# JakubValtar/basisu_rs

Measured on AMD Instinct MI355X. Metric: M 4x4 blocks/s UASTC->BC7 4096x4096, higher is better.
Workload: dtype u8

## Files before the change

basisu_rs_amd/csrc/bu_kernels.hpp:

```cpp
#pragma once
namespace {

constexpr unsigned bu_lds_front(int target) { return target == 1 ? (unsigned)sizeof(BuBc7Tables) : 0u; }
constexpr unsigned bu_lds_table_bytes(int target) { return bu_lds_front(target) + bu_table_bytes(target); }
template <int WGS, int TARGET>
__device__ __forceinline__ void bu_stage_tables_n(uint4* dst, const BuTablesAll* __restrict__ src)
{
    constexpr BuTableRange R = bu_table_range(TARGET);
    constexpr int F = (int)bu_lds_front(TARGET) / 16;
    const uint4* s = reinterpret_cast<const uint4*>(TARGET == 1 ? reinterpret_cast<const void*>(src) : reinterpret_cast<const void*>(&src->t));
    uint4* d = dst;
    for (int i = threadIdx.x; i < F + (int)(R.hi / 16); i += WGS)
        if (i < F || i >= F + (int)(R.lo / 16)) d[i] = s[i];
    if constexpr (R.lo2 < R.hi2) {
        for (int i = F + R.lo2 / 16 + threadIdx.x; i < F + (int)(R.hi2 / 16); i += WGS) d[i] = s[i];
    }
}

__device__ __forceinline__ void bu_report(unsigned long long* status, unsigned long long block, int st)
{
    if (status) (void)__hip_atomic_fetch_min(status, (block << 8) | (unsigned long long)st, __ATOMIC_RELAXED, __HIP_MEMORY_SCOPE_SYSTEM);
}

typedef unsigned int bu_v4u __attribute__((ext_vector_type(4)));
typedef unsigned int bu_v2u __attribute__((ext_vector_type(2)));
__device__ __forceinline__ uint4 bu_ld_stream(const uint4* p)
{
    const bu_v4u r = __builtin_nontemporal_load(reinterpret_cast<const bu_v4u*>(p));
    return make_uint4(r.x, r.y, r.z, r.w);
}
#ifndef BU_ST_MODE
#define BU_ST_MODE 4
#endif
#if BU_ST_MODE == 2
#define BU_ST_BITS " sc1"
#elif BU_ST_MODE == 3
#define BU_ST_BITS " sc0 sc1"
#elif BU_ST_MODE == 4
#define BU_ST_BITS " sc1 nt"
#endif
__device__ __forceinline__ void bu_st_stream(uint4* p, const uint4 v)
{
    bu_v4u r;
    r.x = v.x; r.y = v.y; r.z = v.z; r.w = v.w;
#if BU_ST_MODE == 0
    __builtin_nontemporal_store(r, reinterpret_cast<bu_v4u*>(p));
#elif BU_ST_MODE == 1
    *reinterpret_cast<bu_v4u*>(p) = r;
#else
    asm volatile("global_store_dwordx4 %0, %1, off" BU_ST_BITS "\n\ts_nop 1" ::"v"(p), "v"(r) : "memory");
#endif
}
__device__ __forceinline__ void bu_st_stream(uint2* p, const uint2 v)
{
    bu_v2u r;
    r.x = v.x; r.y = v.y;
#if BU_ST_MODE == 1
    *reinterpret_cast<bu_v2u*>(p) = r;
#else
    __builtin_nontemporal_store(r, reinterpret_cast<bu_v2u*>(p));
#endif
}

template <int TARGET>
__global__ __launch_bounds__(BU_WG) void bu_uastc_kernel(const uint4* __restrict__ in, void* __restrict__ out, size_t n_blocks,
                                                         unsigned bpr, unsigned long long base, unsigned long long* status,
                                                         const BuTablesAll* __restrict__ tables)
{
    __shared__ uint4 t_store[bu_lds_table_bytes(TARGET) / 16];
    BuTables& T = *reinterpret_cast<BuTables*>(t_store + bu_lds_front(TARGET) / 16);
    const size_t stride = (size_t)gridDim.x * BU_WG;
    size_t idx = (size_t)blockIdx.x * BU_WG + threadIdx.x;
    uint4 v = idx < n_blocks ? bu_ld_stream(in + idx) : make_uint4(0, 0, 0, 0);
    bu_stage_tables_n<BU_WG, TARGET>(t_store, tables);
    __syncthreads();
    while (idx < n_blocks) {
        const size_t next = idx + stride;
        const uint4 vn = next < n_blocks ? in[next] : make_uint4(0, 0, 0, 0);
        BuBlk b;
        b.w[0] = v.x;
        b.w[1] = v.y;
        b.w[2] = v.z;
        b.w[3] = v.w;
        const uint32_t mode = T.mode_lut[v.x & 127u];
        uint32_t o[TARGET == BU_TGT_RGBA ? 16 : 4];
#pragma unroll
        for (int i = 0; i < (TARGET == BU_TGT_RGBA ? 16 : 4); i++) o[i] = 0;
        const int st = bu_block_any<TARGET>(T, mode, b, o);
        if (st) {
            bu_report(status, base + idx, st);
#pragma unroll
            for (int i = 0; i < (TARGET == BU_TGT_RGBA ? 16 : 4); i++) o[i] = 0;
        }
        if constexpr (bu_out_words(TARGET) == 2) {
            reinterpret_cast<uint2*>(out)[idx] = make_uint2(o[0], o[1]);
        } else if constexpr (TARGET == BU_TGT_RGBA) {
            const size_t by = idx / bpr, bx = idx - by * bpr;
            uint4* img = reinterpret_cast<uint4*>(out);
#pragma unroll
            for (int r = 0; r < 4; r++) img[(4 * by + r) * (size_t)bpr + bx] = make_uint4(o[4 * r], o[4 * r + 1], o[4 * r + 2], o[4 * r + 3]);
        } else {
            reinterpret_cast<uint4*>(out)[idx] = make_uint4(o[0], o[1], o[2], o[3]);
        }
        v = vn;
        idx = next;
    }
}

__device__ __forceinline__ uint32_t bu_scan32(uint32_t v)
{
    v += (uint32_t)__builtin_amdgcn_update_dpp(0, (int)v, 0x111, 0xf, 0xf, false);
    v += (uint32_t)__builtin_amdgcn_update_dpp(0, (int)v, 0x112, 0xf, 0xf, false);
    v += (uint32_t)__builtin_amdgcn_update_dpp(0, (int)v, 0x114, 0xf, 0xf, false);
    v += (uint32_t)__builtin_amdgcn_update_dpp(0, (int)v, 0x118, 0xf, 0xf, false);
    v += (uint32_t)__builtin_amdgcn_update_dpp(0, (int)v, 0x142, 0xa, 0xf, false);
    return v;
}

struct BuRunDesc {
    const uint4* in;
    void* out;
    uint64_t base;
    uint32_t n;
    uint32_t vshift;
};
struct BuRunTable {
    BuRunDesc run[BU_MULTI_RUNS];
    uint32_t first_tile[BU_MULTI_RUNS + 32];
};
static_assert(sizeof(BuRunDesc) == 32 && sizeof(BuRunTable) <= 3968, "the run table must fit the 4 KiB of kernel arguments beside the other parameters");
struct BuTileDesc {
    const uint4* in;
    void* out;
    uint32_t first;
    uint32_t n;
    uint64_t base;
    uint32_t width;
};
enum { BU_LAYOUT_STRIP = 0, BU_LAYOUT_RECT = 1, BU_LAYOUT_MULTI = 2,
       BU_LAYOUT_MULTI_WHOLE = 3 };
constexpr unsigned BU_TICKET_STRIDE = 32, BU_TICKET_DONE = 8 * BU_TICKET_STRIDE, BU_TICKET_WORDS = 9 * BU_TICKET_STRIDE;
template <int TARGET, int WGS, int BPT, bool PREFETCH, int LAYOUT>
__device__ __forceinline__ void bu_uastc_sorted_body(const uint4* __restrict__ in, void* __restrict__ out, unsigned n_blocks,
                                                     unsigned bpr, unsigned long long base, unsigned long long* status,
                                                     const BuTablesAll* __restrict__ tables, unsigned cus, unsigned tile_rt,
                                                     const BuRunTable* __restrict__ runs, unsigned* __restrict__ ticket = nullptr)
{
    if (cus != 0) {
        constexpr bool ROT = TARGET == BU_TGT_BC7 || TARGET == BU_TGT_ASTC;
        if (blockIdx.x >= 3 * cus) __builtin_amdgcn_s_setprio(ROT ? 1 : 3);
        else if (blockIdx.x >= 2 * cus) __builtin_amdgcn_s_setprio(2);
        else if (blockIdx.x >= cus) __builtin_amdgcn_s_setprio(ROT ? 3 : 1);
    }
    constexpr int BU_WG = WGS, BU_BPT = BPT, BU_TILE = WGS * BPT;
    __shared__ uint4 t_store[bu_lds_table_bytes(TARGET) / 16];
    BuTables& T = *reinterpret_cast<BuTables*>(t_store + bu_lds_front(TARGET) / 16);
    constexpr bool RECT = LAYOUT == BU_LAYOUT_RECT, MULTI = LAYOUT == BU_LAYOUT_MULTI || LAYOUT == BU_LAYOUT_MULTI_WHOLE;
    constexpr bool WHOLE = RECT || LAYOUT == BU_LAYOUT_MULTI_WHOLE;
    constexpr bool BU_ALIAS = TARGET == BU_TGT_RGBA;
    static_assert(!BU_ALIAS || bu_lds_table_bytes(TARGET) + 4 * BU_TILE * 16 + BU_TILE + 1536 <= 80 * 1024,
                  "the RGBA32 workgroup no longer fits twice per CU: shrink BuTables or stage it per target in LDS too");
    __shared__ uint4 sblk_store[BU_ALIAS ? 1 : BU_TILE];
    __shared__ uint4 sout[BU_ALIAS ? 4 * BU_TILE : 1];
    uint4* const sblk = BU_ALIAS ? sout : sblk_store;
    constexpr bool INBLOCK = TARGET == BU_TGT_BC7 || TARGET == BU_TGT_ASTC;
    __shared__ uint8_t sst[INBLOCK ? 16 : BU_TILE];
    __shared__ uint32_t cnt[2][32], next_chunk[2];
    const unsigned tid = threadIdx.x, lane = tid & 63u;
    constexpr bool DYN_TILE = bu_dyn_tile(TARGET, BU_TILE) && LAYOUT != BU_LAYOUT_RECT;
    const unsigned tile_blocks = DYN_TILE ? tile_rt : (unsigned)BU_TILE;
    const unsigned n_tiles = (n_blocks + tile_blocks - 1) / tile_blocks;
    auto in_tile = [&](unsigned l) { return !DYN_TILE || l < tile_blocks; };
    static_assert(!RECT || BU_TILE % BU_RECT_W == 0, "rectangular tiles are BU_RECT_W blocks wide and of fixed size");
    const unsigned tpr = RECT ? bpr / BU_RECT_W : 1u;
    auto tile_xy = [&](unsigned t, unsigned& ty, unsigned& tx) {
        ty = (unsigned)(((unsigned long long)t * tile_rt) >> 32);
        tx = t - ty * tpr;
    };
    auto gidx = [&](unsigned t, unsigned l) {
        if constexpr (RECT) {
            unsigned ty, tx;
            tile_xy(t, ty, tx);
            return ((unsigned)(BU_TILE / BU_RECT_W) * ty + l / BU_RECT_W) * bpr + BU_RECT_W * tx + (l % BU_RECT_W);
        } else {
            return t * tile_blocks + l;
        }
    };
    auto has_block = [&](uint32_t k) { return WHOLE || k < 20u; };
    unsigned tile = blockIdx.x;
    __shared__ uint32_t s_next_tile[2];
    uint32_t my_draw = 0;
    unsigned* const my_counter = ticket ? ticket + (blockIdx.x & 7u) * BU_TICKET_STRIDE : nullptr;
    auto tile_of_draw = [&](uint32_t d) { return gridDim.x + 8u * d + (blockIdx.x & 7u); };
    if (ticket && tid == 0) my_draw = atomicAdd(my_counter, 1u);
    BuTileDesc td = {in, out, 0u, 0u, base, 0u}, tl = td;
    constexpr bool RUNS_IN_LDS = MULTI && PREFETCH;
    __shared__ uint4 s_runs[RUNS_IN_LDS ? sizeof(BuRunTable) / 16 : 1];
    const BuRunTable* R = runs;
    if constexpr (RUNS_IN_LDS) {
        static_assert(sizeof(BuRunTable) % 16 == 0, "copied in 16-byte pieces");
        for (unsigned i = tid; i < sizeof(BuRunTable) / 16; i += WGS) s_runs[i] = reinterpret_cast<const uint4*>(runs)[i];
    }
    auto uni32 = [](uint32_t x) { return (uint32_t)__builtin_amdgcn_readfirstlane((int)x); };
    auto uni64 = [&](uint64_t x) { return (uint64_t)uni32((uint32_t)x) | ((uint64_t)uni32((uint32_t)(x >> 32)) << 32); };
    auto desc_of = [&](unsigned t, BuTileDesc& d) {
        if constexpr (MULTI) {
            if (t < n_tiles) {
                uint32_t r = 0;
#pragma unroll
                for (unsigned c = 0; c < BU_MULTI_RUNS + 32; c += 64) {
                    const uint32_t cnt = (uint32_t)__popcll(__ballot(R->first_tile[c + lane] <= t));
                    if (cnt) r = c + cnt - 1u;
                }
                r = (uint32_t)__builtin_amdgcn_readfirstlane((int)r);
                const BuRunDesc rv = R->run[r];
                const BuRunDesc rd = {reinterpret_cast<const uint4*>(uni64(reinterpret_cast<uint64_t>(rv.in))), reinterpret_cast<void*>(uni64(reinterpret_cast<uint64_t>(rv.out))),
                                      uni64(rv.base), uni32(rv.n), uni32(rv.vshift)};
                const uint32_t lt = t - uni32(R->first_tile[r]);
                if (rd.vshift != BU_RUN_STRIPS) {
                    const uint32_t ty = lt >> rd.vshift, tx = lt & ((1u << rd.vshift) - 1u), width = (uint32_t)BU_RECT_W << rd.vshift;
                    d = BuTileDesc{rd.in, rd.out, (uint32_t)(BU_TILE / BU_RECT_W) * ty * width + (uint32_t)BU_RECT_W * tx, (uint32_t)BU_TILE, rd.base, width};
                } else {
                    const uint32_t first = lt * (uint32_t)BU_TILE, left = rd.n - first;
                    d = BuTileDesc{rd.in, rd.out, first, left < (uint32_t)BU_TILE ? left : (uint32_t)BU_TILE, rd.base, 0u};
                }
            }
        }
    };
    desc_of(tile, td);
    tl = td;
    auto run_idx = [&](const BuTileDesc& d, unsigned l) { return d.first + ((WHOLE || d.width) ? (l / BU_RECT_W) * d.width + (l % BU_RECT_W) : l); };
    auto blk_src = [&](unsigned t, unsigned l) { return MULTI ? tl.in + run_idx(tl, l) : in + gidx(t, l); };
    auto blk_valid = [&](unsigned t, unsigned l) {
        if constexpr (MULTI) return t < n_tiles && (WHOLE || l < tl.n);
        else return RECT ? t < n_tiles : (t < n_tiles && gidx(t, l) < n_blocks && in_tile(l));
    };
    constexpr BuTableRange TR = bu_table_range(TARGET);
    constexpr bool SPLIT = bu_lds_table_bytes(TARGET) > 16384;
    constexpr int TF = (int)bu_lds_front(TARGET) / 16, TV1 = (int)(TR.hi - TR.lo) / 16, TV2 = TR.lo2 < TR.hi2 ? (int)(TR.hi2 - TR.lo2) / 16 : 0;
    constexpr int TVT = TF + TV1 + TV2, TVN = (TVT + WGS - 1) / WGS;
    const uint4* const tsrc = reinterpret_cast<const uint4*>(TARGET == BU_TGT_BC7 ? reinterpret_cast<const void*>(tables) : reinterpret_cast<const void*>(&tables->t));
    auto tdst = [&](int i) { return i < TF ? i : (i < TF + TV1 ? (int)(TR.lo / 16) + i : TF + (int)(TR.lo2 / 16) + (i - TF - TV1)); };
    uint4 tv[TVN];
    if constexpr (!SPLIT) {
#pragma unroll
        for (int k = 0; k < TVN; k++) {
            const int i = k * WGS + (int)tid;
            tv[k] = i < TVT ? tsrc[tdst(i)] : make_uint4(0, 0, 0, 0);
        }
    }
    uint4 v[BU_BPT];
#pragma unroll
    for (int j = 0; j < BU_BPT; j++)
        v[j] = (RECT || blk_valid(tile, j * BU_WG + tid)) ? bu_ld_stream(blk_src(tile, j * BU_WG + tid)) : make_uint4(0, 0, 0, 0);
    if constexpr (!SPLIT) {
#pragma unroll
        for (int k = 0; k < TVN; k++) {
            const int i = k * WGS + (int)tid;
            if (i < TVT) t_store[tdst(i)] = tv[k];
        }
    } else {
#pragma unroll
        for (int k = 0; k < TVN; k++) {
            const int i = k * WGS + (int)tid;
            tv[k] = i < TVT ? tsrc[tdst(i)] : make_uint4(0, 0, 0, 0);
        }
        static_assert(offsetof(BuTables, key_lut) % 4 == 0 && sizeof(T.key_lut[0]) == 128, "the target's key_lut is staged as 32 dwords");
        if (tid < 32) reinterpret_cast<uint32_t*>(T.key_lut[bu_cost_row(TARGET)])[tid] = reinterpret_cast<const uint32_t*>(tables->t.key_lut[bu_cost_row(TARGET)])[tid];
    }
    bool tables_staged = !SPLIT;
    if (tid < 64) (&cnt[0][0])[tid] = 0;
    if (tid < 2) next_chunk[tid] = 0;
    __syncthreads();
    if constexpr (RUNS_IN_LDS) R = reinterpret_cast<const BuRunTable*>(s_runs);
    unsigned par = 0;
    unsigned next_of_loop = 0;
    for (; tile < n_tiles; tile = next_of_loop, par ^= 1u) {
        const unsigned tbase = tile * tile_blocks;
        uint32_t key[BU_BPT], pos[BU_BPT];
        bool uniform = true;
#pragma unroll
        for (int j = 0; j < BU_BPT; j++) {
            const bool valid = WHOLE || (MULTI ? (unsigned)(j * BU_WG) + tid < td.n : (tbase + j * BU_WG + tid < n_blocks && in_tile(j * BU_WG + tid)));
            key[j] = valid ? T.key_lut[bu_cost_row(TARGET)][v[j].x & 127u] : 31u;
            uniform = uniform && (__ballot(key[j] == (uint32_t)__builtin_amdgcn_readfirstlane(key[j])) == ~0ull) && has_block(key[j]);
        }
        if (uniform) {
            uint32_t lead[BU_BPT];
#pragma unroll
            for (int j = 0; j < BU_BPT; j++) lead[j] = lane == 0 ? atomicAdd(&cnt[par][key[j]], 64u) : 0u;
#pragma unroll
            for (int j = 0; j < BU_BPT; j++) pos[j] = (uint32_t)__builtin_amdgcn_readfirstlane(lead[j]) + lane;
        } else {
#pragma unroll
            for (int j = 0; j < BU_BPT; j++) pos[j] = atomicAdd(&cnt[par][key[j]], 1u);
        }
        if (ticket && tid == 0) s_next_tile[par] = tile_of_draw(my_draw);
        if (!tables_staged) {
#pragma unroll
            for (int k = 0; k < TVN; k++) {
                const int i = k * WGS + (int)tid;
                if (i < TVT) t_store[tdst(i)] = tv[k];
            }
            tables_staged = true;
        }
        __syncthreads();
        const uint32_t run_c = lane < 20u ? cnt[par][lane] : 0u;
        const uint32_t run_pk = run_c | (((run_c + 63u) >> 6) << 16);
        const uint32_t run_incl = bu_scan32(run_pk), run_excl = run_incl - run_pk;
        const uint32_t nc = (uint32_t)__builtin_amdgcn_readlane((int)run_incl, 31) >> 16;
        if (tid < 32) cnt[par ^ 1u][tid] = 0;
        if (tid == 0) next_chunk[par ^ 1u] = 0;
        uint32_t dest[BU_BPT];
#pragma unroll
        for (int j = 0; j < BU_BPT; j++) {
            const uint32_t st = (uint32_t)__builtin_amdgcn_ds_bpermute((int)(key[j] << 2), (int)run_excl) & 0xFFFFu;
            dest[j] = has_block(key[j]) ? st + pos[j] : 0u;
            if (has_block(key[j])) sblk[dest[j]] = v[j];
        }
        const unsigned ntile = ticket ? (unsigned)__builtin_amdgcn_readfirstlane((int)s_next_tile[par]) : tile + gridDim.x;
        next_of_loop = ntile;
        uint4 vn[BU_BPT];
        if constexpr (PREFETCH) {
            desc_of(ntile, tl);
#pragma unroll
            for (int j = 0; j < BU_BPT; j++) {
                vn[j] = blk_valid(ntile, j * BU_WG + tid) ? bu_ld_stream(blk_src(ntile, j * BU_WG + tid)) : make_uint4(0, 0, 0, 0);
            }
        }
        if (ticket && tid == 0 && ntile < n_tiles) my_draw = atomicAdd(my_counter, 1u);
        __syncthreads();
        uint32_t c_next = 0;
        if (lane == 0) c_next = atomicAdd(&next_chunk[par], 1u);
        for (;;) {
            const uint32_t c = __builtin_amdgcn_readfirstlane(c_next);
            if (c >= nc) break;
            if (lane == 0) c_next = atomicAdd(&next_chunk[par], 1u);
            const uint32_t r = (uint32_t)__builtin_ctzll(__ballot((run_incl >> 16) > c));
            const uint32_t r_pk = (uint32_t)__builtin_amdgcn_readlane((int)run_pk, (int)r), r_ex = (uint32_t)__builtin_amdgcn_readlane((int)run_excl, (int)r);
            const uint32_t k64 = (c - (r_ex >> 16)) << 6;
            const uint32_t s0 = (r_ex & 0xFFFFu) + k64, left = (r_pk & 0xFFFFu) - k64, count = left < 64u ? left : 64u;
            const bool active = lane < count;
            const uint32_t slot = s0 + (active ? lane : 0u);
            const uint4 bv = sblk[slot];
            BuBlk b;
            b.w[0] = bv.x;
            b.w[1] = bv.y;
            b.w[2] = bv.z;
            b.w[3] = bv.w;
            constexpr int NO = TARGET == BU_TGT_RGBA ? 16 : 4;
            uint32_t o[NO];
#pragma unroll
            for (int i = 0; i < NO; i++) o[i] = 0;
            int st = BU_ST_BAD_MODE;
            if (active) {
                switch (r) {
#define BU_CASE(k) \
    case k: st = bu_block_mode<TARGET, BU_COST_ORDER[bu_cost_row(TARGET)][k]>(T, b, o); break;
                    BU_CASE(0) BU_CASE(1) BU_CASE(2) BU_CASE(3) BU_CASE(4) BU_CASE(5) BU_CASE(6) BU_CASE(7) BU_CASE(8) BU_CASE(9)
                    BU_CASE(10) BU_CASE(11) BU_CASE(12) BU_CASE(13) BU_CASE(14) BU_CASE(15) BU_CASE(16) BU_CASE(17) BU_CASE(18)
#undef BU_CASE
                default: break;
                }
                if constexpr (TARGET == BU_TGT_RGBA) {
#pragma unroll
                    for (int r2 = 0; r2 < 4; r2++) sout[r2 * BU_TILE + slot] = make_uint4(o[4 * r2], o[4 * r2 + 1], o[4 * r2 + 2], o[4 * r2 + 3]);
                    sst[slot] = (uint8_t)st;
                } else if constexpr (INBLOCK) {
                    sblk[slot] = make_uint4(o[0], o[1], o[2], o[3] | (uint32_t)st);
                } else {
                    sblk[slot] = make_uint4(o[0], o[1], o[2], o[3]);
                    sst[slot] = (uint8_t)st;
                }
            }
        }
        __syncthreads();
#pragma unroll
        for (int j = 0; j < BU_BPT; j++) {
            if (has_block(key[j])) {
                const unsigned idx = MULTI ? run_idx(td, j * BU_WG + tid) : gidx(tile, j * BU_WG + tid);
                void* const out = td.out;
                const unsigned long long base = td.base;
                if constexpr (INBLOCK) {
                    uint4 r = sblk[dest[j]];
                    if ((r.x & 0xFFu) == 0u) {
                        bu_report(status, base + idx, (int)r.w);
                        r.w = 0;
                    }
                    bu_st_stream(reinterpret_cast<uint4*>(out) + idx, r);
                    continue;
                }
                const uint32_t st = sst[dest[j]];
                if (st) bu_report(status, base + idx, (int)st);
                if constexpr (TARGET == BU_TGT_RGBA) {
                    unsigned by, bx;
                    if constexpr (RECT) {
                        const unsigned l = j * BU_WG + tid;
                        unsigned ty, tx;
                        tile_xy(tile, ty, tx);
                        by = (unsigned)(BU_TILE / BU_RECT_W) * ty + l / BU_RECT_W;
                        bx = BU_RECT_W * tx + (l % BU_RECT_W);
                    } else {
                        by = idx / bpr;
                        bx = idx - by * bpr;
                    }
                    uint4* img = reinterpret_cast<uint4*>(out);
#pragma unroll
                    for (int r = 0; r < 4; r++) bu_st_stream(img + (size_t)((4 * by + r) * bpr + bx), sout[r * BU_TILE + dest[j]]);
                } else {
                    const uint4 r = sblk[dest[j]];
                    if constexpr (bu_out_words(TARGET) == 2) bu_st_stream(reinterpret_cast<uint2*>(out) + idx, make_uint2(r.x, r.y));
                    else bu_st_stream(reinterpret_cast<uint4*>(out) + idx, r);
                }
            }
        }
        if constexpr (PREFETCH) {
#pragma unroll
            for (int j = 0; j < BU_BPT; j++) v[j] = vn[j];
            td = tl;
        } else {
            desc_of(ntile, tl);
            td = tl;
#pragma unroll
            for (int j = 0; j < BU_BPT; j++) v[j] = blk_valid(ntile, j * BU_WG + tid) ? bu_ld_stream(blk_src(ntile, j * BU_WG + tid)) : make_uint4(0, 0, 0, 0);
        }
    }
    if (ticket && tid == 0) {
        if (atomicAdd(ticket + BU_TICKET_DONE, 1u) == gridDim.x - 1u) {
            for (unsigned k = 0; k < 8; k++) atomicExch(ticket + k * BU_TICKET_STRIDE, 0u);
            atomicExch(ticket + BU_TICKET_DONE, 0u);
        }
    }
}

template <int TARGET, int WGS, int BPT, int MINW, bool PREFETCH, int LAYOUT>
__global__ __launch_bounds__(WGS, MINW) void bu_uastc_sorted_kernel(const uint4* __restrict__ in, void* __restrict__ out, unsigned n_blocks,
                                                                unsigned bpr, unsigned long long base, unsigned long long* status,
                                                                const BuTablesAll* __restrict__ tables, unsigned cus, unsigned tile_rt,
                                                                unsigned* __restrict__ ticket)
{
    static_assert(LAYOUT != BU_LAYOUT_MULTI && LAYOUT != BU_LAYOUT_MULTI_WHOLE, "several runs per launch: bu_uastc_multi_kernel");
    bu_uastc_sorted_body<TARGET, WGS, BPT, PREFETCH, LAYOUT>(in, out, n_blocks, bpr, base, status, tables, cus, tile_rt, nullptr, ticket);
}

constexpr bool bu_multi_etc_2048(int target, int tile) { return bu_etc_family(target) && tile == 2048; }
template <int TARGET, int WGS, int BPT, bool PREFETCH = false, bool WHOLE = false>
__global__ __launch_bounds__(WGS, (TARGET == BU_TGT_ASTC && WGS == 512) ? 8 : bu_multi_etc_2048(TARGET, WGS * BPT) ? 4 : 1) void bu_uastc_multi_kernel(
    const BuRunTable table, unsigned n_tiles, unsigned bpr, unsigned long long* status, const BuTablesAll* __restrict__ tables, unsigned* __restrict__ ticket)
{
    static_assert(WGS * BPT == 1024 || bu_multi_etc_2048(TARGET, WGS * BPT), "the host numbers 1024-block tiles (ETC1 / ETC2 large batches: 2048-block ones)");
    static_assert(sizeof(BuRunTable) + 40 <= 4096, "the run table and the other arguments share the 4 KiB of kernel arguments");
    bu_uastc_sorted_body<TARGET, WGS, BPT, PREFETCH, WHOLE ? BU_LAYOUT_MULTI_WHOLE : BU_LAYOUT_MULTI>(nullptr, nullptr, n_tiles * (unsigned)(WGS * BPT), bpr, 0ull, status, tables, 0u,
                                                                                                        (unsigned)(WGS * BPT), &table, ticket);
}

__global__ void bu_status_reset_kernel(unsigned long long* words, unsigned n)
{
    for (unsigned i = threadIdx.x; i < n; i += blockDim.x) words[i] = ~0ull;
}

struct BuCrcTables {
    uint16_t t[4][256];
    uint16_t pw[256];
};
constexpr unsigned BU_CRC_PIECE = 65536;

__device__ __forceinline__ uint32_t bu_crc_gf_mul(uint32_t a, uint32_t b)
{
    uint32_t r = 0;
#pragma unroll
    for (int i = 15; i >= 0; i--) {
        r <<= 1;
        r ^= (r & 0x10000u) ? 0x11021u : 0u;
        r ^= ((b >> i) & 1u) ? a : 0u;
    }
    return r & 0xFFFFu;
}

__global__ __launch_bounds__(256) void bu_crc16_pieces_kernel(const uint4* __restrict__ data, uint16_t* __restrict__ partial,
                                                              const BuCrcTables* __restrict__ tables)
{
    __shared__ BuCrcTables C;
    __shared__ uint32_t red[4];
    static_assert(sizeof(BuCrcTables) % 16 == 0, "copied in 16-byte pieces");
    for (unsigned i = threadIdx.x; i < sizeof(BuCrcTables) / 16; i += 256) reinterpret_cast<uint4*>(&C)[i] = reinterpret_cast<const uint4*>(tables)[i];
    __syncthreads();
    const uint4* p = data + (size_t)blockIdx.x * (BU_CRC_PIECE / 16) + threadIdx.x * 16;
    uint32_t s = 0;
#pragma unroll 4
    for (int i = 0; i < 16; i++) {
        const uint4 v = p[i];
        const uint32_t w[4] = {v.x, v.y, v.z, v.w};
#pragma unroll
        for (int k = 0; k < 4; k++) {
            const uint32_t x = w[k];
            s = (uint32_t)C.t[3][((s >> 8) ^ x) & 255u] ^ (uint32_t)C.t[2][(s ^ (x >> 8)) & 255u] ^ (uint32_t)C.t[1][(x >> 16) & 255u] ^ (uint32_t)C.t[0][x >> 24];
        }
    }
    uint32_t c = bu_crc_gf_mul(s, C.pw[255u - threadIdx.x]);
#pragma unroll
    for (int d = 32; d >= 1; d >>= 1) c ^= (uint32_t)__shfl_xor((int)c, d);
    if ((threadIdx.x & 63u) == 0) red[threadIdx.x >> 6] = c;
    __syncthreads();
    if (threadIdx.x == 0) partial[blockIdx.x] = (uint16_t)(red[0] ^ red[1] ^ red[2] ^ red[3]);
}

__global__ __launch_bounds__(64) void bu_sleep_kernel(unsigned long long ticks)
{
    const unsigned long long t0 = wall_clock64();
    while (wall_clock64() - t0 < ticks) __builtin_amdgcn_s_sleep(32);
}

template <int WG, int EPT>
__global__ __launch_bounds__(WG) void bu_copy_kernel(const uint4* __restrict__ in, uint4* __restrict__ out, size_t n)
{
    const size_t base = (size_t)blockIdx.x * (WG * EPT) + threadIdx.x;
    uint4 v[EPT];
#pragma unroll
    for (int k = 0; k < EPT; k++) {
        const size_t i = base + (size_t)k * WG;
        if (i < n) v[k] = bu_ld_stream(in + i);
    }
#pragma unroll
    for (int k = 0; k < EPT; k++) {
        const size_t i = base + (size_t)k * WG;
        if (i < n) {
            bu_v4u r;
            r.x = v[k].x; r.y = v[k].y; r.z = v[k].z; r.w = v[k].w;
            __builtin_nontemporal_store(r, reinterpret_cast<bu_v4u*>(out + i));
        }
    }
}

}
```

Baseline: 186,300.

## Use inline-asm async prefetch loads with counted vmcnt waits and SGPR-base addressing

For the whole-tile prefetch path on BC7/ASTC, next-tile block loads and the ticket atomic are issued as inline asm, so the compiler no longer inserts a full vmcnt(0) wait. A single s_waitcnt vmcnt(BPT) after the output stores then waits for the loads without waiting for the stores to drain. Loads and stores now use a scalar base plus a 32-bit per-lane offset in the global address space, which saves VGPRs and 64-bit address arithmetic. The approach depends on an exact count of outstanding memory ops, so any store that is added or skipped would break correctness.

```diff
diff --git a/basisu_rs_amd/csrc/bu_kernels.hpp b/basisu_rs_amd/csrc/bu_kernels.hpp
--- a/basisu_rs_amd/csrc/bu_kernels.hpp
+++ b/basisu_rs_amd/csrc/bu_kernels.hpp
@@ -24,9 +24,15 @@
 
 typedef unsigned int bu_v4u __attribute__((ext_vector_type(4)));
 typedef unsigned int bu_v2u __attribute__((ext_vector_type(2)));
+#define BU_GLOBAL __attribute__((address_space(1)))
 __device__ __forceinline__ uint4 bu_ld_stream(const uint4* p)
 {
-    const bu_v4u r = __builtin_nontemporal_load(reinterpret_cast<const bu_v4u*>(p));
+    const bu_v4u r = __builtin_nontemporal_load((const BU_GLOBAL bu_v4u*)p);
+    return make_uint4(r.x, r.y, r.z, r.w);
+}
+__device__ __forceinline__ uint4 bu_ld_stream(uint64_t base, uint32_t off)
+{
+    const bu_v4u r = __builtin_nontemporal_load((const BU_GLOBAL bu_v4u*)((const BU_GLOBAL char*)base + off));
     return make_uint4(r.x, r.y, r.z, r.w);
 }
 #ifndef BU_ST_MODE
@@ -44,9 +50,9 @@
     bu_v4u r;
     r.x = v.x; r.y = v.y; r.z = v.z; r.w = v.w;
 #if BU_ST_MODE == 0
-    __builtin_nontemporal_store(r, reinterpret_cast<bu_v4u*>(p));
+    __builtin_nontemporal_store(r, (BU_GLOBAL bu_v4u*)p);
 #elif BU_ST_MODE == 1
-    *reinterpret_cast<bu_v4u*>(p) = r;
+    *(BU_GLOBAL bu_v4u*)p = r;
 #else
     asm volatile("global_store_dwordx4 %0, %1, off" BU_ST_BITS "\n\ts_nop 1" ::"v"(p), "v"(r) : "memory");
 #endif
@@ -56,10 +62,40 @@
     bu_v2u r;
     r.x = v.x; r.y = v.y;
 #if BU_ST_MODE == 1
-    *reinterpret_cast<bu_v2u*>(p) = r;
+    *(BU_GLOBAL bu_v2u*)p = r;
 #else
-    __builtin_nontemporal_store(r, reinterpret_cast<bu_v2u*>(p));
+    __builtin_nontemporal_store(r, (BU_GLOBAL bu_v2u*)p);
 #endif
+}
+__device__ __forceinline__ void bu_st_stream(uint64_t base, uint32_t off, const uint4 v)
+{
+#if BU_ST_MODE < 2
+    bu_st_stream(reinterpret_cast<uint4*>(base + off), v);
+#else
+    bu_v4u r;
+    r.x = v.x; r.y = v.y; r.z = v.z; r.w = v.w;
+    asm volatile("global_store_dwordx4 %0, %1, %2" BU_ST_BITS "\n\ts_nop 1" ::"v"(off), "v"(r), "s"(base) : "memory");
+#endif
+}
+constexpr bool BU_COUNTED_WAITS = BU_ST_MODE >= 2;
+__device__ __forceinline__ void bu_ld_stream_async(bu_v4u& r, uint64_t base, uint32_t off)
+{
+    asm volatile("global_load_dwordx4 %0, %1, %2 nt" : "+v"(r) : "v"(off), "s"(base) : "memory");
+}
+__device__ __forceinline__ void bu_atomic_inc_async(uint32_t& r, const unsigned* counter)
+{
+    asm volatile("global_atomic_add %0, %1, %2, %3 sc0" : "+v"(r) : "v"(0u), "v"(1u), "s"(counter) : "memory");
+}
+template <int N>
+__device__ __forceinline__ void bu_wait_vm()
+{
+    static_assert(N >= 0 && N < 64, "vmcnt is a 6-bit counter");
+    asm volatile("s_waitcnt vmcnt(%0)" ::"n"(N) : "memory");
+}
+template <typename V>
+__device__ __forceinline__ void bu_arrived(V& r)
+{
+    asm volatile("" : "+v"(r));
 }
 
 template <int TARGET>
@@ -230,7 +266,16 @@
     desc_of(tile, td);
     tl = td;
     auto run_idx = [&](const BuTileDesc& d, unsigned l) { return d.first + ((WHOLE || d.width) ? (l / BU_RECT_W) * d.width + (l % BU_RECT_W) : l); };
-    auto blk_src = [&](unsigned t, unsigned l) { return MULTI ? tl.in + run_idx(tl, l) : in + gidx(t, l); };
+    auto tile_off = [&](const BuTileDesc& d, unsigned l) { return (((WHOLE || d.width) ? (l / BU_RECT_W) * d.width + (l % BU_RECT_W) : l)) * 16u; };
+    auto ld_base = [&]() { return MULTI ? reinterpret_cast<uint64_t>(tl.in) + (uint64_t)tl.first * 16u : reinterpret_cast<uint64_t>(in); };
+    auto ld_off = [&](unsigned t, unsigned l) { return MULTI ? tile_off(tl, l) : gidx(t, l) * 16u; };
+    auto ld_blk = [&](unsigned t, unsigned l) {
+        if constexpr (MULTI) return bu_ld_stream(ld_base(), ld_off(t, l));
+        else return bu_ld_stream(in + gidx(t, l));
+    };
+    constexpr bool COUNTED = BU_COUNTED_WAITS && PREFETCH && WHOLE && (TARGET == BU_TGT_BC7 || TARGET == BU_TGT_ASTC);
+    static_assert(!COUNTED || (bu_out_words(TARGET) == 4 && bu_lds_table_bytes(TARGET) <= 16384), "one 16-byte asm store per block; tables staged before the loop (no table load is pending inside it)");
+    constexpr int STORES_PER_TILE = BPT;
     auto blk_valid = [&](unsigned t, unsigned l) {
         if constexpr (MULTI) return t < n_tiles && (WHOLE || l < tl.n);
         else return RECT ? t < n_tiles : (t < n_tiles && gidx(t, l) < n_blocks && in_tile(l));
@@ -252,7 +297,7 @@
     uint4 v[BU_BPT];
 #pragma unroll
     for (int j = 0; j < BU_BPT; j++)
-        v[j] = (RECT || blk_valid(tile, j * BU_WG + tid)) ? bu_ld_stream(blk_src(tile, j * BU_WG + tid)) : make_uint4(0, 0, 0, 0);
+        v[j] = (RECT || blk_valid(tile, j * BU_WG + tid)) ? ld_blk(tile, j * BU_WG + tid) : make_uint4(0, 0, 0, 0);
     if constexpr (!SPLIT) {
 #pragma unroll
         for (int k = 0; k < TVN; k++) {
@@ -273,6 +318,16 @@
     if (tid < 2) next_chunk[tid] = 0;
     __syncthreads();
     if constexpr (RUNS_IN_LDS) R = reinterpret_cast<const BuRunTable*>(s_runs);
+    if constexpr (COUNTED) {
+#pragma unroll
+        for (int j = 0; j < BU_BPT; j++) {
+            bu_arrived(v[j].x);
+            bu_arrived(v[j].y);
+            bu_arrived(v[j].z);
+            bu_arrived(v[j].w);
+        }
+        bu_arrived(my_draw);
+    }
     unsigned par = 0;
     unsigned next_of_loop = 0;
     for (; tile < n_tiles; tile = next_of_loop, par ^= 1u) {
@@ -321,14 +376,28 @@
         const unsigned ntile = ticket ? (unsigned)__builtin_amdgcn_readfirstlane((int)s_next_tile[par]) : tile + gridDim.x;
         next_of_loop = ntile;
         uint4 vn[BU_BPT];
+        bu_v4u vna[BU_BPT];
         if constexpr (PREFETCH) {
             desc_of(ntile, tl);
-#pragma unroll
-            for (int j = 0; j < BU_BPT; j++) {
-                vn[j] = blk_valid(ntile, j * BU_WG + tid) ? bu_ld_stream(blk_src(ntile, j * BU_WG + tid)) : make_uint4(0, 0, 0, 0);
+            if constexpr (COUNTED) {
+#pragma unroll
+                for (int j = 0; j < BU_BPT; j++) vna[j] = bu_v4u{0u, 0u, 0u, 0u};
+                if (blk_valid(ntile, 0)) {
+                    const uint64_t b = ld_base();
+#pragma unroll
+                    for (int j = 0; j < BU_BPT; j++) bu_ld_stream_async(vna[j], b, ld_off(ntile, j * BU_WG + tid));
+                }
+            } else {
+#pragma unroll
+                for (int j = 0; j < BU_BPT; j++) {
+                    vn[j] = blk_valid(ntile, j * BU_WG + tid) ? ld_blk(ntile, j * BU_WG + tid) : make_uint4(0, 0, 0, 0);
+                }
             }
         }
-        if (ticket && tid == 0 && ntile < n_tiles) my_draw = atomicAdd(my_counter, 1u);
+        if (ticket && tid == 0 && ntile < n_tiles) {
+            if constexpr (COUNTED) bu_atomic_inc_async(my_draw, my_counter);
+            else my_draw = atomicAdd(my_counter, 1u);
+        }
         __syncthreads();
         uint32_t c_next = 0;
         if (lane == 0) c_next = atomicAdd(&next_chunk[par], 1u);
@@ -375,6 +444,8 @@
             }
         }
         __syncthreads();
+        const uint64_t st_base = reinterpret_cast<uint64_t>(td.out) + (MULTI ? (uint64_t)td.first * 16u : 0u);
+        auto st16 = [&](unsigned l, unsigned idx, const uint4 r) { bu_st_stream(st_base, MULTI ? tile_off(td, l) : idx * 16u, r); };
 #pragma unroll
         for (int j = 0; j < BU_BPT; j++) {
             if (has_block(key[j])) {
@@ -387,7 +458,7 @@
                         bu_report(status, base + idx, (int)r.w);
                         r.w = 0;
                     }
-                    bu_st_stream(reinterpret_cast<uint4*>(out) + idx, r);
+                    st16(j * BU_WG + tid, idx, r);
                     continue;
                 }
                 const uint32_t st = sst[dest[j]];
@@ -410,11 +481,21 @@
                 } else {
                     const uint4 r = sblk[dest[j]];
                     if constexpr (bu_out_words(TARGET) == 2) bu_st_stream(reinterpret_cast<uint2*>(out) + idx, make_uint2(r.x, r.y));
-                    else bu_st_stream(reinterpret_cast<uint4*>(out) + idx, r);
+                    else st16(j * BU_WG + tid, idx, r);
                 }
             }
         }
-        if constexpr (PREFETCH) {
+        if constexpr (COUNTED) {
+            static_assert(WHOLE && STORES_PER_TILE == BU_BPT, "the counted wait stands for the unconditional stores of phase D, one per block");
+            bu_wait_vm<STORES_PER_TILE>();
+#pragma unroll
+            for (int j = 0; j < BU_BPT; j++) {
+                bu_arrived(vna[j]);
+                v[j] = make_uint4(vna[j].x, vna[j].y, vna[j].z, vna[j].w);
+            }
+            bu_arrived(my_draw);
+            td = tl;
+        } else if constexpr (PREFETCH) {
 #pragma unroll
             for (int j = 0; j < BU_BPT; j++) v[j] = vn[j];
             td = tl;
@@ -422,7 +503,7 @@
             desc_of(ntile, tl);
             td = tl;
 #pragma unroll
-            for (int j = 0; j < BU_BPT; j++) v[j] = blk_valid(ntile, j * BU_WG + tid) ? bu_ld_stream(blk_src(ntile, j * BU_WG + tid)) : make_uint4(0, 0, 0, 0);
+            for (int j = 0; j < BU_BPT; j++) v[j] = blk_valid(ntile, j * BU_WG + tid) ? ld_blk(ntile, j * BU_WG + tid) : make_uint4(0, 0, 0, 0);
         }
     }
     if (ticket && tid == 0) {
```

Result: faster. 191,400, median of 6 (+2.7%).

## Compute next tile keys before issuing stores; use global address-space loads and stores

Applied to the files above, without the earlier changes.

For prefetching multi-run BC7 (and some ASTC) configurations, the loop now reads the LUT keys for the next tile and the next drawn tile index before issuing the current tile's output stores. The aim is for the stores to go out last, so the following loop iteration does not stall on store counters or on a dependent LDS or atomic read. Loads and stores are also cast to the global address space so the compiler emits global rather than flat instructions. The change adds register pressure for the buffered results and a hand-written waitcnt, and it duplicates the store path.

```diff
diff --git a/basisu_rs_amd/csrc/bu_kernels.hpp b/basisu_rs_amd/csrc/bu_kernels.hpp
--- a/basisu_rs_amd/csrc/bu_kernels.hpp
+++ b/basisu_rs_amd/csrc/bu_kernels.hpp
@@ -29,6 +29,14 @@
     const bu_v4u r = __builtin_nontemporal_load(reinterpret_cast<const bu_v4u*>(p));
     return make_uint4(r.x, r.y, r.z, r.w);
 }
+__device__ __forceinline__ uint4 bu_ld_stream_global(const uint4* p)
+{
+    typedef const bu_v4u __attribute__((address_space(1))) * bu_global_v4u;
+    const bu_v4u r = __builtin_nontemporal_load((bu_global_v4u)p);
+    return make_uint4(r.x, r.y, r.z, r.w);
+}
+typedef bu_v4u __attribute__((address_space(1))) * bu_global_out_v4u;
+typedef bu_v2u __attribute__((address_space(1))) * bu_global_out_v2u;
 #ifndef BU_ST_MODE
 #define BU_ST_MODE 4
 #endif
@@ -44,9 +52,9 @@
     bu_v4u r;
     r.x = v.x; r.y = v.y; r.z = v.z; r.w = v.w;
 #if BU_ST_MODE == 0
-    __builtin_nontemporal_store(r, reinterpret_cast<bu_v4u*>(p));
+    __builtin_nontemporal_store(r, (bu_global_out_v4u)p);
 #elif BU_ST_MODE == 1
-    *reinterpret_cast<bu_v4u*>(p) = r;
+    *(bu_global_out_v4u)p = r;
 #else
     asm volatile("global_store_dwordx4 %0, %1, off" BU_ST_BITS "\n\ts_nop 1" ::"v"(p), "v"(r) : "memory");
 #endif
@@ -56,9 +64,9 @@
     bu_v2u r;
     r.x = v.x; r.y = v.y;
 #if BU_ST_MODE == 1
-    *reinterpret_cast<bu_v2u*>(p) = r;
+    *(bu_global_out_v2u)p = r;
 #else
-    __builtin_nontemporal_store(r, reinterpret_cast<bu_v2u*>(p));
+    __builtin_nontemporal_store(r, (bu_global_out_v2u)p);
 #endif
 }
 
@@ -231,6 +239,7 @@
     tl = td;
     auto run_idx = [&](const BuTileDesc& d, unsigned l) { return d.first + ((WHOLE || d.width) ? (l / BU_RECT_W) * d.width + (l % BU_RECT_W) : l); };
     auto blk_src = [&](unsigned t, unsigned l) { return MULTI ? tl.in + run_idx(tl, l) : in + gidx(t, l); };
+    auto ld_blk = [&](unsigned t, unsigned l) { return MULTI ? bu_ld_stream_global(blk_src(t, l)) : bu_ld_stream(blk_src(t, l)); };
     auto blk_valid = [&](unsigned t, unsigned l) {
         if constexpr (MULTI) return t < n_tiles && (WHOLE || l < tl.n);
         else return RECT ? t < n_tiles : (t < n_tiles && gidx(t, l) < n_blocks && in_tile(l));
@@ -252,7 +261,7 @@
     uint4 v[BU_BPT];
 #pragma unroll
     for (int j = 0; j < BU_BPT; j++)
-        v[j] = (RECT || blk_valid(tile, j * BU_WG + tid)) ? bu_ld_stream(blk_src(tile, j * BU_WG + tid)) : make_uint4(0, 0, 0, 0);
+        v[j] = (RECT || blk_valid(tile, j * BU_WG + tid)) ? ld_blk(tile, j * BU_WG + tid) : make_uint4(0, 0, 0, 0);
     if constexpr (!SPLIT) {
 #pragma unroll
         for (int k = 0; k < TVN; k++) {
@@ -275,14 +284,30 @@
     if constexpr (RUNS_IN_LDS) R = reinterpret_cast<const BuRunTable*>(s_runs);
     unsigned par = 0;
     unsigned next_of_loop = 0;
+    constexpr bool STORES_LAST = PREFETCH && MULTI && (TARGET == BU_TGT_BC7 || (TARGET == BU_TGT_ASTC && WGS == 256 && WHOLE));
+    auto key_of = [&](const BuTileDesc& d, unsigned l, uint32_t x) { return (WHOLE || l < d.n) ? (uint32_t)T.key_lut[bu_cost_row(TARGET)][x & 127u] : 31u; };
+    uint32_t next_key[STORES_LAST ? BU_BPT : 1];
+    uint32_t drawn_tile = 0;
+    if constexpr (STORES_LAST) {
+        if (tile < n_tiles) {
+#pragma unroll
+            for (int j = 0; j < BU_BPT; j++) next_key[j] = key_of(td, j * BU_WG + tid, v[j].x);
+        }
+        if (ticket && tid == 0) drawn_tile = tile_of_draw(my_draw);
+        __builtin_amdgcn_s_waitcnt(0x0F70);
+    }
     for (; tile < n_tiles; tile = next_of_loop, par ^= 1u) {
-        const unsigned tbase = tile * tile_blocks;
+        [[maybe_unused]] const unsigned tbase = tile * tile_blocks;
         uint32_t key[BU_BPT], pos[BU_BPT];
         bool uniform = true;
 #pragma unroll
         for (int j = 0; j < BU_BPT; j++) {
-            const bool valid = WHOLE || (MULTI ? (unsigned)(j * BU_WG) + tid < td.n : (tbase + j * BU_WG + tid < n_blocks && in_tile(j * BU_WG + tid)));
-            key[j] = valid ? T.key_lut[bu_cost_row(TARGET)][v[j].x & 127u] : 31u;
+            if constexpr (STORES_LAST) {
+                key[j] = next_key[j];
+            } else {
+                const bool valid = WHOLE || (MULTI ? (unsigned)(j * BU_WG) + tid < td.n : (tbase + j * BU_WG + tid < n_blocks && in_tile(j * BU_WG + tid)));
+                key[j] = valid ? T.key_lut[bu_cost_row(TARGET)][v[j].x & 127u] : 31u;
+            }
             uniform = uniform && (__ballot(key[j] == (uint32_t)__builtin_amdgcn_readfirstlane(key[j])) == ~0ull) && has_block(key[j]);
         }
         if (uniform) {
@@ -295,7 +320,7 @@
 #pragma unroll
             for (int j = 0; j < BU_BPT; j++) pos[j] = atomicAdd(&cnt[par][key[j]], 1u);
         }
-        if (ticket && tid == 0) s_next_tile[par] = tile_of_draw(my_draw);
+        if (ticket && tid == 0) s_next_tile[par] = STORES_LAST ? drawn_tile : tile_of_draw(my_draw);
         if (!tables_staged) {
 #pragma unroll
             for (int k = 0; k < TVN; k++) {
@@ -325,7 +350,7 @@
             desc_of(ntile, tl);
 #pragma unroll
             for (int j = 0; j < BU_BPT; j++) {
-                vn[j] = blk_valid(ntile, j * BU_WG + tid) ? bu_ld_stream(blk_src(ntile, j * BU_WG + tid)) : make_uint4(0, 0, 0, 0);
+                vn[j] = blk_valid(ntile, j * BU_WG + tid) ? ld_blk(ntile, j * BU_WG + tid) : make_uint4(0, 0, 0, 0);
             }
         }
         if (ticket && tid == 0 && ntile < n_tiles) my_draw = atomicAdd(my_counter, 1u);
@@ -375,6 +400,29 @@
             }
         }
         __syncthreads();
+        if constexpr (STORES_LAST) {
+            uint4 r[BU_BPT];
+            bool has[BU_BPT];
+            auto out_idx = [&](int j) { return run_idx(td, j * BU_WG + tid); };
+#pragma unroll
+            for (int j = 0; j < BU_BPT; j++) {
+                has[j] = has_block(key[j]);
+                if (has[j]) {
+                    r[j] = sblk[dest[j]];
+                    if ((r[j].x & 0xFFu) == 0u) {
+                        bu_report(status, td.base + out_idx(j), (int)r[j].w);
+                        r[j].w = 0;
+                    }
+                }
+            }
+#pragma unroll
+            for (int j = 0; j < BU_BPT; j++) next_key[j] = key_of(tl, j * BU_WG + tid, vn[j].x);
+            drawn_tile = tile_of_draw(my_draw);
+            asm volatile("" : "+v"(drawn_tile));
+#pragma unroll
+            for (int j = 0; j < BU_BPT; j++)
+                if (has[j]) bu_st_stream(reinterpret_cast<uint4*>(td.out) + out_idx(j), r[j]);
+        } else {
 #pragma unroll
         for (int j = 0; j < BU_BPT; j++) {
             if (has_block(key[j])) {
@@ -414,6 +462,7 @@
                 }
             }
         }
+        }
         if constexpr (PREFETCH) {
 #pragma unroll
             for (int j = 0; j < BU_BPT; j++) v[j] = vn[j];
@@ -422,7 +471,7 @@
             desc_of(ntile, tl);
             td = tl;
 #pragma unroll
-            for (int j = 0; j < BU_BPT; j++) v[j] = blk_valid(ntile, j * BU_WG + tid) ? bu_ld_stream(blk_src(ntile, j * BU_WG + tid)) : make_uint4(0, 0, 0, 0);
+            for (int j = 0; j < BU_BPT; j++) v[j] = blk_valid(ntile, j * BU_WG + tid) ? ld_blk(ntile, j * BU_WG + tid) : make_uint4(0, 0, 0, 0);
         }
     }
     if (ticket && tid == 0) {
```

After: 189,800 before, 192,700 after (median of 6 runs). +1.5%, better.
